# pascalPost/turbomesh

Hardware: AMD Instinct MI355X
Metric: nodes smoothed/sec (elliptic sweeps, 4096^2 blocks) + achieved HBM GB/s (higher is better)
Workload: dtype f64

## Files before the change

turbomesh_amd/csrc/tm_kernels.h:

```cpp
#pragma once
#include <hip/hip_runtime.h>
#include <cstdint>
#include "tm_edge_types.h"
#include <vector>

namespace tmh {

enum ApplyMode : int {
    MODE_RAW = 0,
    MODE_SCALED = 1,
    MODE_RESID = 2,
    MODE_RELAX = 3,
    MODE_DIAG_COPY = 4,
    MODE_DIAG_SUM9 = 5,
    MODE_DIAG_NOSTORE = 6,
    MODE_DIAG_NOLOAD = 7,
    MODE_DIAG_MATH = 8,
    MODE_MG_RESID = 9,
    MODE_MG_SMOOTH = 10,
    MODE_MG_FIRST2 = 11
};
enum DotMode : int {
    DOT_NONE = 0,
    DOT_AUX = 1,
// ... 29 lines not shown
int apply_block_nwg(int ni, int nj, int rows = 0);
int apply_block_nwg_overlap(int ni, int nj, int rows = 0);
void tune_apply(int rows_per_chunk, int unroll, int pipe, int nt);
hipError_t launch_apply_block(const ApplyBlock& a, int mode, int dot, hipStream_t stream);
constexpr int APPLY_BATCH_MAX = 8;
struct ApplyBatch {
    ApplyBlock b[APPLY_BATCH_MAX];
    int RI[APPLY_BATCH_MAX], nSG[APPLY_BATCH_MAX], nRC[APPLY_BATCH_MAX];
    int start[APPLY_BATCH_MAX];
    int n;
};
hipError_t launch_apply_blocks(const ApplyBlock* blocks, int n, int mode, int dot, hipStream_t stream);

struct Relax2Block {
    const double2* in;
    double2* mid;
    double2* out;
    int ni, nj;
    double omega;
    double* partials;
    const int32_t* border;
    int nborder;
    int store_nt = 1;
    int dyn;
};
bool relax2_supported(int ni, int nj);
int relax2_rows_per_chunk(int ni, int nj);
int relax2_block_nwg(int ni, int nj, int rows_per_chunk);
std::vector<int32_t> relax2_border_tiles(int ni, int nj, int rows_per_chunk, int dyn);
enum Relax2Subset { R2_ALL = 0, R2_BORDER = 1, R2_INSIDE_A = 2, R2_INSIDE_B = 3, R2_INSIDE = 4 };
constexpr long long QUEUE_WAIT_TICKS = 30LL * 100000000LL;
constexpr long long QUEUE_SELF_TEST_TICKS = 500000LL;
struct QueueWait {
    const uint32_t* counter = nullptr;
    uint32_t target = 0;
    uint32_t* error = nullptr;
    long long limit_ticks = QUEUE_WAIT_TICKS;
};
hipError_t launch_relax2_block(const Relax2Block& a, int rows_per_chunk, int dot, int subset, hipStream_t stream, size_t lds_bytes = 0,
                               const QueueWait* wait = nullptr);
struct Relax2Batch {
    Relax2Block b[8];
    int RI[8], nSG[8], nRC[8], start[8];
    int n;
};
hipError_t launch_relax2_blocks(const Relax2Block* blocks, const int* rows_per_chunk, int n, int dot, int subset, hipStream_t stream,
                                size_t lds_bytes = 0, const QueueWait* wait = nullptr);
void tune_fuse_rows(int rows);
bool relax3_supported(int ni, int nj);
int relax3_rows_per_chunk(int ni, int nj);
void relax3_rows_for_launch(const int* ni, const int* nj, int n, int* rows, bool beside_chain);
int relax3_block_nwg(int ni, int nj, int rows_per_chunk);
hipError_t launch_relax3_blocks(const Relax2Block* blocks, const int* rows_per_chunk, int n, int dot, hipStream_t stream);

hipError_t launch_edge_levels3(const FusedLevelsDev& F, const EdgeRowsDev& e1, const EdgeRowsDev& e2, const EdgeRowsDev& e3, const double2* x, double2* m,
                               double2* m2, double2* out, const double2* pq, double omega, int dot, double* partials ,
                               hipStream_t stream);
hipError_t launch_edge_rows(const EdgeRowsDev& e, const double2* in, const double2* xk, const double2* pq, const double2* aux,
                            double2* out, double omega, int mode, int dot, double* partials, hipStream_t stream, uint32_t* signal = nullptr);
hipError_t launch_apply_edge_blocks(const ApplyBlock* blocks, int n, int mode, int dot, const EdgeRowsDev& e, const double2* in, const double2* xk,
                                    const double2* pq, const double2* aux, double2* out, double* edge_partials, hipStream_t stream);
constexpr int VK_NONE = 0, VK_S = 1, VK_P = 2, VK_R = 3, VK_S2 = 4, VK_PRO = 5;
struct VirtualIn {
    int kind;
    const double2 *in, *in2, *in3, *aux;
    double2* pout;
    const double2* in4 = nullptr;
    double2* rout = nullptr;
    double2* uio = nullptr;
};
hipError_t launch_apply_virtual(const ApplyBlock* blocks, int n, const EdgeRowsDev& e, const VirtualIn& V, const double2* xk, const double2* pq, double2* out,
                                double* edge_partials, const LazyScalars& scal, hipStream_t stream, bool overlap = false);
hipError_t launch_edge_rhs(const EdgeRowsDev& e, const double2* xk, const double2* pq, double2* rhs_out, int scaled,
                           double* partials , hipStream_t stream);

hipError_t launch_queue_signal(uint32_t* counter, hipStream_t stream);
hipError_t launch_queue_wait(const uint32_t* counter, uint32_t target, uint32_t* error, hipStream_t stream, long long limit_ticks = QUEUE_WAIT_TICKS);
hipError_t launch_queue_signal_wait(uint32_t* counter, const uint32_t* other, uint32_t target, uint32_t* error, hipStream_t stream,
                                    long long limit_ticks = QUEUE_WAIT_TICKS);

hipError_t launch_assemble_interior(const double2* xk, const double2* pq, int ni, int nj, const int32_t* row_ptr ,
                                    double* vx, double* vy, hipStream_t stream);
hipError_t launch_assemble_edge(const EdgeRowsDev& e, const double2* xk, const double2* pq, const int32_t* row_ptr, double* vx, double* vy, hipStream_t stream);
hipError_t launch_csr_product(int64_t n, const int32_t* row_ptr, const int32_t* col, const double* vx, const double* vy, const double2* in, double2* out,
                              hipStream_t stream);
hipError_t launch_delay_us(double us, hipStream_t stream);

hipError_t launch_finalize(const double* partials, int nwg, double* red, hipStream_t stream);

struct KrylovScalars {
    double rho[2], rho_old[2], alpha[2], omega[2], beta[2];
    double tol2[2];
    double rr[2];
    double rr0[2];
    int32_t done[2];
    int32_t early[2];
    int32_t iters;
    int32_t _pad;
};
constexpr int VEC_BLOCK = 256;
int vec_nwg(int64_t n);
enum ScalarStep : int { STEP_INIT = 0, STEP_SIGMA = 1, STEP_SS = 2, STEP_TSTT = 3, STEP_RHO = 4, STEP_TOL = 5, STEP_SS_TSTT = 6, STEP_INIT2 = 7, STEP_A2 = 8, STEP_B2 = 9 };
hipError_t launch_scalar_update(KrylovScalars* S, const double* red, int step, hipStream_t stream, double rtol = 0.0, double atol = 0.0);
hipError_t launch_finalize_scalar(const double* partials, int nwg, double* red, KrylovScalars* S, int step, hipStream_t stream, double rtol = 0.0,
                                  double atol = 0.0);
struct LazyStep {
// ... 106 lines not shown
```

turbomesh_amd/csrc/tm_kernels.hip:

```cpp
#include "tm_kernels.h"
#include "tm_devutil.hpp"
#include "tm_refmath.h"
#include <cstdlib>
#include <type_traits>

namespace tmh {

__device__ __forceinline__ double lane_prev(double edge, double v) {
    int2 o = __builtin_bit_cast(int2, edge), s = __builtin_bit_cast(int2, v), r;
    r.x = __builtin_amdgcn_update_dpp(o.x, s.x, 0x138 , 0xf, 0xf, false);
    r.y = __builtin_amdgcn_update_dpp(o.y, s.y, 0x138, 0xf, 0xf, false);
    return __builtin_bit_cast(double, r);
}
__device__ __forceinline__ double lane_next(double edge, double v) {
    int2 o = __builtin_bit_cast(int2, edge), s = __builtin_bit_cast(int2, v), r;
    r.x = __builtin_amdgcn_update_dpp(o.x, s.x, 0x130 , 0xf, 0xf, false);
    r.y = __builtin_amdgcn_update_dpp(o.y, s.y, 0x130, 0xf, 0xf, false);
    return __builtin_bit_cast(double, r);
}
__device__ __forceinline__ double2 lane_prev(double2 edge, double2 v) { return make_double2(lane_prev(edge.x, v.x), lane_prev(edge.y, v.y)); }
__device__ __forceinline__ double2 lane_next(double2 edge, double2 v) { return make_double2(lane_next(edge.x, v.x), lane_next(edge.y, v.y)); }

__device__ __forceinline__ double2 lane_prev0(double2 v) {
    int4 s = __builtin_bit_cast(int4, v), r;
// ... 838 lines not shown
            __builtin_amdgcn_raw_buffer_store_b128(__builtin_bit_cast(v4i32, o), out_rsrc,
                                                   static_cast<int>(row_live ? lane_off + static_cast<unsigned>((i - t.i0) * nj * 16) : OOB_VOFFSET), 0,
                                                   (NT & 1) ? 2 : 0);
            if (DOT == DOT_DELTA) {
                if (!(live_lane && row_live)) d3 = zero;
                accumulate<DOT_DELTA>(acc, S2[A1].c, o, d3);
            }
        }
#pragma unroll
        for (int u = 0; u < U; ++u) pc[u] = pn[u];
    };
    static_assert(U == 3, "the phases below assume three steps per group");
    group(0, 0);
    group(U, 1);
    for (int tb = 2 * U; tb < nsteps; tb += U) group(tb, 2);
}

template <int DOT, int U, int NT, bool W1>
__device__ __forceinline__ void relax3_tile(const Relax2Block& a, int RI, int nSG, int nRC, int bid) {
    const int lane = threadIdx.x & 63;
    const int wave = threadIdx.x >> 6;
    const int total = nSG * nRC;
    const int q8 = total >> 3, rem = total & 7, xcd = bid & 7, k8 = bid >> 3;
    const int logical = (xcd < rem) ? xcd * (q8 + 1) + k8 : rem * (q8 + 1) + (xcd - rem) * q8 + k8;
    const int rc = logical / nSG;
    const int sg = logical - rc * nSG;
    const int ni = a.ni, nj = a.nj;
    Relax2Tile t;
    t.c0 = (sg * 4 + wave) * R3_W;
    t.c = t.c0 - R3_H + lane;
    t.out_lane = (lane >= R3_H) && (lane < 64 - R3_H) && (t.c >= 1) && (t.c <= nj - 2);
    t.i0 = 1 + rc * RI;
    t.i1 = min(t.i0 + RI, ni - 1);
    double acc[MAX_PARTIALS] = {0.0, 0.0, 0.0, 0.0};
    if (t.c0 <= nj - 2 && t.i0 < t.i1) {
        const bool inside = (t.c0 - R3_H >= 1) && (t.c0 - R3_H + 63 <= nj - 2) && (t.i0 - 3 >= 1) && (t.i1 + 2 <= ni - 2);
        if (inside) relax3_strip<DOT, U, NT, W1, true>(a, t, acc);
        else relax3_strip<DOT, U, NT, W1, false>(a, t, acc);
    }
    if (DOT != DOT_NONE) block_partials<256, dot_columns(DOT)>(acc, a.partials + static_cast<size_t>(logical) * MAX_PARTIALS);
}
template <int DOT, int U, int NT, bool W1>
__global__ __launch_bounds__(256, TM_R3_WAVES) void k_relax3(Relax2Block a, int RI, int nSG, int nRC) {
    relax3_tile<DOT, U, NT, W1>(a, RI, nSG, nRC, blockIdx.x);
}
template <int DOT, int U, int NT, bool W1>
__global__ __launch_bounds__(256) void k_relax3_batch(Relax2Batch B) {
    int k = 0;
#pragma unroll
    for (int q = 1; q < APPLY_BATCH_MAX; ++q)
        if (q < B.n && static_cast<int>(blockIdx.x) >= B.start[q]) k = q;
    relax3_tile<DOT, U, NT, W1>(B.b[k], B.RI[k], B.nSG[k], B.nRC[k], static_cast<int>(blockIdx.x) - B.start[k]);
}
static int g_fuse3_rows = 0;
void relax3_rows_for_launch(const int* ni, const int* nj, int n, int* rows, bool beside_chain) {
    static const int forced = [] { const char* e = std::getenv("TM_FUSE3_ROWS"); return e ? std::atoi(e) : 0; }();
    if (forced > 0 || g_fuse3_rows > 0) {
        for (int k = 0; k < n; ++k) rows[k] = std::max(1, std::min(forced > 0 ? forced : g_fuse3_rows, ni[k] - 2));
        return;
    }
    static int slots = 0;
    if (slots == 0) {
        int dev = 0, cus = 0;
        if (hipGetDevice(&dev) != hipSuccess || hipDeviceGetAttribute(&cus, hipDeviceAttributeMultiprocessorCount, dev) != hipSuccess || cus <= 0) cus = 256;
        slots = 3 * cus;
    }
    static const int heights[] = {38, 26, 14, 8};
    const long need = static_cast<long>(slots) * (beside_chain ? 9 : 6);
    int RI = 8;
    for (const int h : heights) {
        long total = 0;
        for (int k = 0; k < n; ++k) {
            const int nstrips = (nj[k] - 1 + R3_W - 1) / R3_W, nSG = (nstrips + 3) / 4, interior = ni[k] - 2, r = std::max(1, std::min(h, interior));
            total += static_cast<long>(nSG) * ((interior + r - 1) / r);
        }
        RI = h;
        if (total * 10 >= need) break;
    }
    for (int k = 0; k < n; ++k) rows[k] = std::max(1, std::min(RI, ni[k] - 2));
}
int relax3_rows_per_chunk(int ni, int nj) {
    int r = 0;
    relax3_rows_for_launch(&ni, &nj, 1, &r, false);
    return r;
}
bool relax3_supported(int ni, int nj) { return ni >= 7 && nj >= 7 && nj <= (1 << 20); }
int relax3_block_nwg(int ni, int nj, int RI) {
    const int nstrips = (nj - 1 + R3_W - 1) / R3_W;
    return ((nstrips + 3) / 4) * ((ni - 2 + RI - 1) / RI);
}
hipError_t launch_relax3_blocks(const Relax2Block* blocks, const int* rows_per_chunk, int n, int dot, hipStream_t st) {
    for (int first = 0; first < n; first += APPLY_BATCH_MAX) {
        Relax2Batch B;
        B.n = 0;
        int total = 0;
        bool w1 = true;
        const bool nts = blocks[first].store_nt != 0;
        for (int k = first; k < n && B.n < APPLY_BATCH_MAX; ++k) {
            const int q = B.n++;
            B.b[q] = blocks[k];
            B.RI[q] = rows_per_chunk[k];
            B.nSG[q] = ((blocks[k].nj - 1 + R3_W - 1) / R3_W + 3) / 4;
            B.nRC[q] = (blocks[k].ni - 2 + B.RI[q] - 1) / B.RI[q];
            B.start[q] = total;
            total += B.nSG[q] * B.nRC[q];
            w1 = w1 && blocks[k].omega == 1.0;
        }
        for (int q = B.n; q < APPLY_BATCH_MAX; ++q) B.start[q] = total;
        if (total == 0) continue;
        const dim3 grid(total), block(256);
#define TM_R3(KERNEL, ...)                                                                                                   \
    do {                                                                                                                     \
        if (dot == DOT_DELTA) {                                                                                              \
            if (w1 && nts) hipLaunchKernelGGL((KERNEL<DOT_DELTA, R3_U, 1, true>), grid, block, 0, st, __VA_ARGS__);          \
            else if (w1) hipLaunchKernelGGL((KERNEL<DOT_DELTA, R3_U, 0, true>), grid, block, 0, st, __VA_ARGS__);            \
            else hipLaunchKernelGGL((KERNEL<DOT_DELTA, R3_U, 1, false>), grid, block, 0, st, __VA_ARGS__);                   \
        } else {                                                                                                             \
            if (w1 && nts) hipLaunchKernelGGL((KERNEL<DOT_NONE, R3_U, 1, true>), grid, block, 0, st, __VA_ARGS__);           \
            else if (w1) hipLaunchKernelGGL((KERNEL<DOT_NONE, R3_U, 0, true>), grid, block, 0, st, __VA_ARGS__);             \
            else hipLaunchKernelGGL((KERNEL<DOT_NONE, R3_U, 1, false>), grid, block, 0, st, __VA_ARGS__);                    \
        }                                                                                                                    \
    } while (0)
        static const bool force_batch = [] { const char* e = std::getenv("TM_R3_FORCE_BATCH"); return e && std::atoi(e) != 0; }();
        if (B.n == 1 && !force_batch) TM_R3(k_relax3, B.b[0], B.RI[0], B.nSG[0], B.nRC[0]);
        else TM_R3(k_relax3_batch, B);
#undef TM_R3
        const hipError_t rc = hipGetLastError();
        if (rc != hipSuccess) return rc;
    }
    return hipSuccess;
}

constexpr int MG_RST_W = 58;
struct MgMetric {
    double G11, G22, mhG12, m2D, D, rinv;
};
__device__ __forceinline__ MgMetric mg_metric(double2 dxi, double2 det) {
    MgMetric m;
    m.G11 = fma(dxi.x, dxi.x, dxi.y * dxi.y);
    m.G22 = fma(det.x, det.x, det.y * det.y);
    const double G12 = fma(dxi.x, det.x, dxi.y * det.y);
    m.D = m.G11 + m.G22;
    m.m2D = -2.0 * m.D;
    m.mhG12 = -0.5 * G12;
    m.rinv = recip_diag(m.D, m.m2D);
    return m;
}
template <bool HAS_PQ>
__device__ __forceinline__ double2 mg_scaled_row(const MgMetric& g, const Row3& m, const Row3& c, const Row3& p, double P, double Q) {
    double ax = p.c.x + m.c.x, ay = p.c.y + m.c.y;
    double bx = c.h.x, by = c.h.y;
    if (HAS_PQ) {
        const double hP = 0.5 * P, hQ = 0.5 * Q;
        ax = fma(hP, p.c.x - m.c.x, ax);
        ay = fma(hP, p.c.y - m.c.y, ay);
        bx = fma(hQ, c.e.x, bx);
        by = fma(hQ, c.e.y, by);
    }
    const double kx = p.e.x - m.e.x;
    const double ky = p.e.y - m.e.y;
    double sx = g.G22 * ax, sy = g.G22 * ay;
    sx = fma(g.G11, bx, sx);
    sy = fma(g.G11, by, sy);
    sx = fma(g.m2D, c.c.x, sx);
    sy = fma(g.m2D, c.c.y, sy);
    sx = fma(g.mhG12, kx, sx);
    sy = fma(g.mhG12, ky, sy);
    return make_double2(sx * g.rinv, sy * g.rinv);
}

template <int KIND, bool HAS_PQ, bool PRO, bool RST, int U>
__device__ __forceinline__ void mg_pair_strip(const MgPairArgs& a, const Relax2Tile& t) {
    static_assert(!RST || KIND == 1, "the restriction rides behind the residual");
    const int ni = a.ni, nj = a.nj;
    const int cc = min(max(t.c, 0), nj - 1);
    const double2 zero = make_double2(0.0, 0.0);
    auto at = [&](int row) { return static_cast<size_t>(min(max(row, 0), ni - 1)) * nj + cc; };
    const bool perim_col = (t.c <= 0) || (t.c >= nj - 1);
    const bool col_in = (t.c >= 1) && (t.c <= nj - 2);
    const int nrows = t.i1 - t.i0;
    const __amdgpu_buffer_rsrc_t out_rsrc = __builtin_amdgcn_make_buffer_rsrc(a.out + static_cast<size_t>(t.i0) * nj, 0, nrows * nj * 16, 0x00020000);
    const __amdgpu_buffer_rsrc_t out2_rsrc =
        __builtin_amdgcn_make_buffer_rsrc((KIND == 1 ? a.out2 : a.out) + static_cast<size_t>(t.i0) * nj, 0, nrows * nj * 16, 0x00020000);
// ... 1804 lines not shown
```

turbomesh_amd/csrc/tm_smoother.cpp:

```cpp
#include "tm_smoother.hpp"
#include "tm_api_util.hpp"
#include "tm_ilu.hpp"
#include "tm_refine.hpp"
#include "tm_quality_dev.hpp"
#include <algorithm>
#include <atomic>
#include <chrono>
#include <cmath>
#include <cstdio>
#include <cstdlib>
#include <cstring>
#include <map>
#include <unordered_map>

namespace tmh {

void hip_check(hipError_t e, const char* what) {
    if (e != hipSuccess) throw TmError(TM_E_HIP, std::string(what) + ": " + hipGetErrorString(e));
}
#define HIPCHK(x) hip_check((x), #x)

std::atomic<int> g_multirank_handles{0};
tm_log_fn g_log_sink = nullptr;
void* g_log_ctx = nullptr;
// ... 400 lines not shown
        return 0;
    };
    apply_rows = shortest_rows(false);
    vk_overlap = vk_able && lp.n_owned >= 50000 && lp.n_owned <= 12000000;
    if (vk_overlap && launch_wgs(apply_rows, false) <= 256 && launch_wgs(shortest_rows(true), true) > 256) vk_overlap = false;
    if (const char* e = std::getenv("TM_VK_OVERLAP")) vk_overlap = vk_able && std::atoi(e) != 0;
    if (vk_overlap) apply_rows = shortest_rows(true);
    if (vk_able && !apply_rows && lp.owned_blocks.size() > 1) apply_rows = 24;
    if (!apply_rows && opt.inner == TM_INNER_RELAX) apply_rows = 6;
    if (const char* e = std::getenv("TM_APPLY_ROWS")) apply_rows = std::max(0, std::atoi(e));
    poff.clear();
    int off = 0;
    for (int64_t b : lp.owned_blocks) {
        poff.push_back(off);
        off += apply_block_nwg(static_cast<int>(topo.ni[b]), static_cast<int>(topo.nj[b]), apply_rows);
    }
    poff_edge = off;
    off += edge_wg;
    nwg_apply = off;
    if (fuse_pairs) {
        poff2.clear();
        rows2.clear();
        int off2 = 0;
        for (int64_t b : lp.owned_blocks) {
            const int bi = static_cast<int>(topo.ni[b]), bj = static_cast<int>(topo.nj[b]);
            poff2.push_back(off2);
            rows2.push_back(relax2_rows_per_chunk(bi, bj));
            off2 += relax2_block_nwg(bi, bj, rows2.back());
            const std::vector<int32_t> ids = relax2_border_tiles(bi, bj, rows2.back(), dyn_mask[poff2.size() - 1]);
            border_n.push_back(static_cast<int>(ids.size()));
            border_ids.push_back(static_cast<const int32_t*>(upload_table(ids.data(), ids.size() * 4)));
        }
        poff2_edge = off2;
        nwg_apply2 = off2 + edge_nf.nwg;
    }
    pipelined_single = fuse_pairs && !(has_hooks && (lp.send_ids.size() > 0 || !lp.ghost_gid.empty())) && edge_nf.nrows > 0 && lp.n_owned >= (1 << 21);
    if (const char* e = std::getenv("TM_SINGLE_PIPELINED")) pipelined_single = pipelined_single && std::atoi(e) != 0;
    fuse_triples = fuse_pairs && edge_nf.nrows == 0 && !(has_hooks && (!lp.send_ids.empty() || !lp.ghost_gid.empty()));
    if (const char* e = std::getenv("TM_FUSE_3")) fuse_triples = fuse_triples && std::atoi(e) != 0;
    if (fuse_triples || triples_coupled) {
        poff3.clear();
        rows3.clear();
        int off3 = 0;
        rows3 = relax3_rows_of_owned_blocks();
        for (size_t k = 0; k < lp.owned_blocks.size(); ++k) {
            const int64_t b = lp.owned_blocks[k];
            const int bi = static_cast<int>(topo.ni[b]), bj = static_cast<int>(topo.nj[b]);
            if (!relax3_supported(bi, bj)) fuse_triples = false;
            poff3.push_back(off3);
            off3 += relax3_block_nwg(bi, bj, rows3[k]);
        }
        nwg_apply3 = off3;
    }
    nwg_vec = vec_nwg(n_owned);
    const int nwg3_all = fuse_triples ? nwg_apply3 : (triples_coupled ? nwg_apply3 + std::max(edge_L[2].nwg, fused_levels.nstrips) : 0);
    if (vk_overlap) {
        int off_ov = 0;
        for (int64_t b : lp.owned_blocks) {
            poff_ov.push_back(off_ov);
            off_ov += apply_block_nwg_overlap(static_cast<int>(topo.ni[b]), static_cast<int>(topo.nj[b]), apply_rows);
        }
        poff_edge_ov = off_ov;
        nwg_apply_ov = off_ov + edge.nwg;
    }
    if (vk_able && std::max(nwg_apply, nwg_apply_ov) <= 512) nwg_vec = std::min(nwg_vec, 512);
    lazy = !has_hooks && opt.inner != TM_INNER_RELAX && std::max(std::max(nwg_apply, nwg_apply_ov), nwg_vec) <= 512 && !(opt.flags & TM_OPT_EAGER_SCALARS);
    const int nwg_refine = refine() ? csr_nwg(n_owned) : 0;
    const uint64_t npart = static_cast<uint64_t>(std::max(std::max(std::max(std::max(std::max(nwg_apply, nwg_apply_ov), nwg_apply2), nwg3_all), nwg_vec), nwg_refine)) * MAX_PARTIALS;
    fuse_s = !has_hooks && opt.inner == TM_INNER_BICGSTAB && !(opt.flags & TM_OPT_EAGER_SCALARS);
    fuse_p = fuse_s;
    if (const char* e = std::getenv("TM_FUSE_P")) fuse_p = fuse_p && std::atoi(e) != 0;
    fuse2 = fuse_p;
    if (const char* e = std::getenv("TM_FUSE_2")) fuse2 = fuse2 && std::atoi(e) != 0;
    if (fuse_p) {
        p_alt = vec();
        v_alt = vec();
    }
    if (fuse2) r_alt = vec();
    const int rows = static_cast<int>(npart / MAX_PARTIALS);
    const struct {
        const char* what;
        int nwg;
    } producers[] = {{"operator", nwg_apply},
                     {"operator (overlapping strips)", nwg_apply_ov},
                     {"sweep pairs", nwg_apply2},
                     {"sweep triples", nwg3_all},
                     {"vector kernels", nwg_vec},
                     {"GMRES Gram-Schmidt", (opt.inner == TM_INNER_GMRES || reference()) ? vec_nwg(n_owned) : 0},
                     {"perimeter-row right-hand side", opt.inner != TM_INNER_RELAX ? edge.nwg : 0},
                     {"refinement step", nwg_refine}};
    if (std::getenv("TM_DEBUG_RUNS"))
        std::fprintf(stderr, "[tm] partial-sum rows: %d allocated; operator %d, overlapping strips %d, pairs %d, triples %d, vector kernels %d (vec_nwg %d)\n", rows,
                     nwg_apply, nwg_apply_ov, nwg_apply2, nwg3_all, nwg_vec, vec_nwg(n_owned));
    for (const auto& q : producers)
        if (q.nwg > rows)
            throw TmError(TM_E_HIP, std::string("internal: the ") + q.what + " launch has " + std::to_string(q.nwg) + " workgroups, the partial-sum buffer " +
                                        std::to_string(rows) + " rows");
    return npart;
}

void Smoother::alloc_reductions(uint64_t npart) {
    partials_guard = false;
    if (const char* e = std::getenv("TM_PARTIALS_GUARD")) partials_guard = std::atoi(e) != 0;
    const uint64_t nguard = partials_guard ? GUARD_DOUBLES : 0;
    for (int k = 0; k < (lazy ? 3 : 1); ++k) part_buf[k] = arena.alloc_n<double>(npart + nguard);
    partials = part_buf[0];
    red = arena.alloc_n<double>(MAX_PARTIALS + nguard);
    if (partials_guard) {
// ... 932 lines not shown
    }
    return rows;
}

void Smoother::ensure_side() {
    if (side) return;
    int least = 0, greatest = 0;
    HIPCHK(hipDeviceGetStreamPriorityRange(&least, &greatest));
    HIPCHK(hipStreamCreateWithPriority(&side, hipStreamNonBlocking, greatest));
    HIPCHK(hipEventCreateWithFlags(&ev_to_side, hipEventDisableTiming));
    HIPCHK(hipEventCreateWithFlags(&ev_to_main, hipEventDisableTiming));
    HIPCHK(hipEventCreateWithFlags(&ev_inside[0], hipEventDisableTiming));
    HIPCHK(hipEventCreateWithFlags(&ev_inside[1], hipEventDisableTiming));
    if (pair_sync_events) queue_ordering = ORDER_EVENTS_REQUESTED;
    else queue_ordering = queue_self_test() ? ORDER_COUNTERS : ORDER_EVENTS_SELF_TEST;
}

bool Smoother::queue_self_test() {
    HIPCHK(hipStreamSynchronize(stream));
    HIPCHK(hipStreamSynchronize(side));
    uint32_t* a = sync_flags + 8;
    uint32_t* b = sync_flags + 9;
    uint32_t* err = sync_flags + 10;
    HIPCHK(hipMemsetAsync(sync_flags + 8, 0, sizeof(uint32_t) * 4, stream));
    HIPCHK(hipStreamSynchronize(stream));
    HIPCHK(launch_queue_signal_wait(a, b, 1u, err, stream, QUEUE_SELF_TEST_TICKS));
    HIPCHK(launch_queue_signal_wait(b, a, 1u, err, side, QUEUE_SELF_TEST_TICKS));
    HIPCHK(hipStreamSynchronize(stream));
    HIPCHK(hipStreamSynchronize(side));
    uint32_t h[4] = {0, 0, 0, 0};
    HIPCHK(hipMemcpy(h, sync_flags + 8, sizeof(h), hipMemcpyDeviceToHost));
    return h[2] == 0u && h[0] == 1u && h[1] == 1u;
}

bool Smoother::use_counters() {
    if (queue_ordering == ORDER_EVENTS_REQUESTED || queue_ordering == ORDER_EVENTS_SELF_TEST) return false;
    if (g_multirank_handles.load() > 1) {
        queue_ordering = ORDER_EVENTS_SHARED_PROCESS;
        return false;
    }
    queue_ordering = ORDER_COUNTERS;
    return true;
}

void Smoother::warm_transport() {
    if (transport_warm) return;
    transport_warm = true;
    if (!(has_hooks && (n_send > 0 || n_ghost > 0))) return;
    exchange(X, side);
    exchange_finish(side);
    HIPCHK(hipStreamSynchronize(side));
}

void Smoother::relax_triple(bool want_partials) {
    const int dot = want_partials ? DOT_DELTA : DOT_NONE;
    std::vector<Relax2Block> blocks(lp.owned_blocks.size());
    for (size_t k = 0; k < lp.owned_blocks.size(); ++k) {
        const int64_t b = lp.owned_blocks[k];
        const int64_t ls = lp.local_start[k];
        Relax2Block& a = blocks[k];
        a.in = X + ls;
        a.mid = nullptr;
        a.out = U + ls;
        a.ni = static_cast<int>(topo.ni[b]);
        a.nj = static_cast<int>(topo.nj[b]);
        a.omega = opt.omega;
        a.dyn = 0;
        a.store_nt = relax2_store_nt ? 1 : 0;
        a.border = nullptr;
        a.nborder = 0;
        a.partials = partials + static_cast<size_t>(poff3[k]) * MAX_PARTIALS;
    }
    profiled([&]() { HIPCHK(launch_relax3_blocks(blocks.data(), rows3.data(), static_cast<int>(blocks.size()), dot, stream)); }, true, stream);
    std::swap(X, U);
}

void Smoother::relax_triples_coupled(uint64_t ntriples, bool want_partials_last) {
    ensure_side();
    const bool use_flags = use_counters();
    uint32_t* chain_done = sync_flags;
    uint32_t* inside_done = sync_flags + 1;
    uint32_t* sync_err = sync_flags + 2;
    if (use_flags) HIPCHK(hipMemsetAsync(sync_flags, 0, sizeof(uint32_t) * 4, stream));
    fence(stream, side, ev_to_side);
    warm_transport();
    std::vector<Relax2Block> blocks(lp.owned_blocks.size());
    for (uint64_t q = 0; q < ntriples; ++q) {
        const int dot = (q + 1 == ntriples && want_partials_last) ? DOT_DELTA : DOT_NONE;
        for (size_t k = 0; k < lp.owned_blocks.size(); ++k) {
            const int64_t b = lp.owned_blocks[k];
            const int64_t ls = lp.local_start[k];
            Relax2Block& a = blocks[k];
            a.in = X + ls;
            a.mid = nullptr;
            a.out = U + ls;
            a.ni = static_cast<int>(topo.ni[b]);
            a.nj = static_cast<int>(topo.nj[b]);
            a.omega = opt.omega;
            a.dyn = dyn_mask[k];
            a.store_nt = relax2_store_nt ? 1 : 0;
            a.border = nullptr;
            a.nborder = 0;
            a.partials = partials + static_cast<size_t>(poff3[k]) * MAX_PARTIALS;
        }
        if (q > 0) {
            if (use_flags) HIPCHK(launch_queue_signal_wait(inside_done, chain_done, static_cast<uint32_t>(q), sync_err, stream));
            else HIPCHK(hipStreamWaitEvent(stream, ev_to_main, 0));
        }
        profiled([&]() { HIPCHK(launch_relax3_blocks(blocks.data(), rows3.data(), static_cast<int>(blocks.size()), dot, stream)); }, true, stream);
        if (!use_flags) HIPCHK(hipEventRecord(ev_inside[q & 1], stream));
        if (q > 0) {
            if (use_flags) HIPCHK(launch_queue_signal_wait(chain_done, inside_done, static_cast<uint32_t>(q), sync_err, side));
            else HIPCHK(hipStreamWaitEvent(side, ev_inside[(q - 1) & 1], 0));
        }
        exchange(X, side);
        exchange_finish(side);
        if (levels_fused) {
            HIPCHK(launch_edge_levels3(fused_levels, edge_L[0], edge_L[1], edge_L[2], X, M, M2, U, PQ, opt.omega, dot,
                                       partials + static_cast<size_t>(nwg_apply3) * MAX_PARTIALS, side));
        } else {
            HIPCHK(launch_edge_rows(edge_L[0], X, X, PQ, nullptr, M, opt.omega, MODE_RELAX, DOT_NONE, partials, side));
            HIPCHK(launch_edge_rows(edge_L[1], M, M, PQ, nullptr, M2, opt.omega, MODE_RELAX, DOT_NONE, partials, side));
            HIPCHK(launch_edge_rows(edge_L[2], M2, M2, PQ, nullptr, U, opt.omega, MODE_RELAX, dot, partials + static_cast<size_t>(nwg_apply3) * MAX_PARTIALS, side));
        }
        if (q + 1 < ntriples && !use_flags) HIPCHK(hipEventRecord(ev_to_main, side));
        std::swap(X, U);
// ... 53 lines not shown
            w.counter = inside_done;
            w.target = inside_upto;
            w.error = sync_err;
            relax2_launch(R2_BORDER, true, dot, side, &w);
        } else {
            if (inside_upto > 0) wait_inside(inside_upto);
            relax2_launch(R2_BORDER, true, dot, side);
        }
    };
    int dot = (npairs == 1 && want_partials_last) ? DOT_DELTA : DOT_NONE;
    fence(stream, side, ev_to_side);
    warm_transport();
    exchange_on_side(X);
    edge_on_side(e1, X, M, DOT_NONE);
    relax2_launch(R2_INSIDE, false, dot);
    if (!use_flags || npairs == 1) signal_inside();
    border_pass(0, dot);
    for (uint64_t k = 0; k < npairs; ++k) {
        const bool announce = k + 1 < npairs;
        if (use_flags && announce) {
            edge_on_side(edge_nf, M, U, dot, border_done);
            n_border += 1;
        } else {
            edge_on_side(edge_nf, M, U, dot);
            if (announce) signal_border();
        }
        std::swap(X, U);
        if (k + 1 == npairs) {
            fence(side, stream, ev_to_main);
            break;
        }
        dot = (k + 2 == npairs && want_partials_last) ? DOT_DELTA : DOT_NONE;
        if (use_flags) {
            HIPCHK(launch_queue_signal_wait(inside_done, border_done, n_border, sync_err, stream));
            n_inside += 1;
        } else {
            wait_border();
        }
        relax2_launch(R2_INSIDE, false, dot);
        if (!use_flags) signal_inside();
        exchange_on_side(X);
        edge_on_side(e1, X, M, DOT_NONE);
        border_pass(static_cast<uint32_t>(k + 1), dot);
    }
    if (use_flags) {
        HIPCHK(hipMemcpyAsync(h_flags, sync_flags, sizeof(uint32_t) * 4, hipMemcpyDeviceToHost, stream));
        flags_pending = true;
    }
}

void Smoother::relax_sweeps(uint64_t n, tm_stats& st) {
    int last_nwg = nwg_apply;
    uint64_t k = 0;
    if ((fuse_triples || triples_coupled) && n >= 3) {
        const uint64_t ntriples = n / 3;
        if (fuse_triples) {
            for (uint64_t q = 0; q < ntriples; ++q) relax_triple(q + 1 == ntriples && n % 3 == 0);
            last_nwg = nwg_apply3;
        } else {
            relax_triples_coupled(ntriples, n % 3 == 0);
            last_nwg = nwg_apply3 + (levels_fused ? fused_levels.nstrips : edge_L[2].nwg);
        }
        k = 3 * ntriples;
        st.operator_sweeps += k;
        outer_done += k;
    }
    if (fuse_pairs && n - k >= 2) {
        const uint64_t npairs = (n - k) / 2;
        const bool last_is_pair = (n - k) % 2 == 0;
        if ((has_hooks && (n_send > 0 || n_ghost > 0)) || pipelined_single) {
            relax_pairs_pipelined(npairs, last_is_pair);
        } else {
            for (uint64_t q = 0; q < npairs; ++q) relax_pair(q + 1 == npairs && last_is_pair);
        }
        k += 2 * npairs;
        st.operator_sweeps += 2 * npairs;
        outer_done += 2 * npairs;
        last_nwg = nwg_apply2;
    }
    for (; k < n; ++k) {
        last_nwg = nwg_apply;
        if (white && outer_done > 0) white_launch(1);
        apply(X, U, MODE_RELAX, DOT_DELTA, nullptr, X, opt.omega);
        std::swap(X, U);
        st.operator_sweeps += 1;
        outer_done += 1;
    }
    if (profile && prof_open) {
        profile_close(stream);
        prof_phase = 0;
    }
    if (n) {
        reduce(last_nwg);
        HIPCHK(hipMemcpyAsync(h_red, red, sizeof(double) * MAX_PARTIALS, hipMemcpyDeviceToHost, stream));
        sync();
        if (flags_pending) {
            flags_pending = false;
            const bool timed_out = h_flags[2] != 0 || h_flags[6] != 0;
            h_flags[2] = h_flags[6] = 0;
            if (timed_out) throw TmError(TM_E_HIP, "a device-side dependency between the interior pass and the chain of a sweep pair / triple was not met within its time limit");
        }
        st.last_dx2 = h_red[0];
        st.last_dy2 = h_red[1];
        st.last_residual = (h_red[0] + h_red[1]) * (h_red[0] + h_red[1]);
        st.scaled_residual_rms = std::sqrt((h_red[0] + h_red[1]) / (2.0 * static_cast<double>(dof_global))) / opt.omega;
    }
}

void Smoother::iterate(uint64_t iterations, tm_stats* stats) {
    const auto t0 = std::chrono::steady_clock::now();
    tm_stats st;
    std::memset(&st, 0, sizeof(st));
    const tm_log_fn sink = g_log_sink;
    if (opt.inner == TM_INNER_RELAX && !sink) {
        relax_sweeps(iterations, st);
        st.outer_iterations = iterations;
    } else {
        for (uint64_t n = 0; n < iterations; ++n) {
// ... 279 lines not shown
```

turbomesh_amd/csrc/tm_smoother.hpp:

```cpp
#pragma once
#include "../../include/tm_hip.h"
#include <cstdlib>
#include "tm_edge_tables.hpp"
#include "tm_kernels.h"
#include "tm_multigrid.hpp"
#include "tm_plan.hpp"
#include <cmath>
#include <atomic>
#include <memory>
#include <string>
#include <functional>
#include <vector>

namespace tmh {

struct TmError : std::runtime_error {
    int code;
    TmError(int c, const std::string& m) : std::runtime_error(m), code(c) {}
};
void hip_check(hipError_t e, const char* what);
extern std::atomic<int> g_multirank_handles;
extern tm_log_fn g_log_sink;
extern void* g_log_ctx;

// ... 41 lines not shown
    std::vector<BlockMG> mg;
    bool use_mg = false;
    bool mg_perimeter_step = false;
    bool mg_dirichlet = false;
    std::vector<hipStream_t> mg_streams;
    std::vector<hipEvent_t> mg_join;
    hipEvent_t mg_fork = nullptr;
    int mg_perimeter_sweeps = 2;
    void precondition(const double2* in, double2* out);
    void precondition_probe_host(const double* f, double* z, double* f_after);
    double2* M = nullptr;
    double2* M2 = nullptr;
    bool fuse_pairs = false;
    bool relax2_store_nt = true;
    bool pair_sync_events = false;
    size_t inside_lds = 0;
    EdgeRowsDev edge;
    std::vector<double> h_rhs;
    struct RhsTable {
        double* dev = nullptr;
        std::vector<const double*> src;
    };
    std::vector<RhsTable> rhs_tables;
    EdgeRowsDev edge_nf;
    EdgeRowsDev edge_nf_g;
    std::vector<int> dyn_mask;
    std::vector<const int32_t*> border_ids;
    std::vector<int> border_n;
    void prefill_fixed();
    double* partials = nullptr;
    double* red = nullptr;
    KrylovScalars* S = nullptr;
    KrylovScalars* h_S = nullptr;
    bool pipelined_poll = false, poll_open = false;
    KrylovScalars* h_poll[2] = {nullptr, nullptr};
    hipEvent_t ev_poll[2] = {nullptr, nullptr};
    uint64_t poll_it[2] = {0, 0}, poll_iters = 0;
    int poll_slot = 0;
    int poll_done(uint64_t it, bool final);
    double stall_best[2] = {0.0, 0.0};
    uint64_t stall_since = 0, stall_window = 4000;
    bool stalled = false;
    double* h_red = nullptr;
    bool vk_overlap = false;
    std::vector<int> poff_ov;
    int poff_edge_ov = 0, nwg_apply_ov = 0;
    std::vector<int> poff;
    int poff_edge = 0, nwg_apply = 0, nwg_vec = 0;
    std::vector<int> poff2, rows2;
    int poff2_edge = 0, nwg_apply2 = 0;
    std::vector<int> poff3, rows3;
    int nwg_apply3 = 0;
    bool fuse_triples = false;
    bool triples_coupled = false;
    EdgeRowsDev edge_L[3];
    bool levels_fused = false;
    FusedLevelsDev fused_levels;
    bool pipelined_single = false;
    int32_t* d_send_ids = nullptr;
    double2* d_send_buf = nullptr;
    int64_t n_send = 0;
    bool white = false;
    ConnShifts white_le{};
    uint64_t outer_done = 0;
    int profile = 0;
    std::vector<hipEvent_t> ev_start, ev_stop;
    size_t ev_used = 0;
    uint64_t prof_launches = 0;
    uint64_t prof_timed = 0;
    uint64_t prof_open = 0;
    uint64_t prof_phase = 0;
    void profile_close(hipStream_t on);
    void profile_read(double* ms_total, uint64_t* launches, uint64_t* timed);

    void create(const tm_mesh_desc* mesh, const tm_solver_opt* o, const tm_control_fn* c, const tm_comm_hooks* h, void* strm,
                bool measure);
    void upload(const tm_mesh_desc* mesh);
    void download(const tm_mesh_desc* mesh);
    void iterate(uint64_t iterations, tm_stats* stats);
    bool iterate_until(uint64_t max_iterations, double tol, tm_stats* stats);
    bool iterate_until_update(uint64_t max_iterations, double tol, tm_stats* stats);
    double stop_tol = 0.0;
    void apply_host(const double* in_xy, double* out_xy, int scaled);
    uint64_t assemble_csr_host(int32_t* Ap, int32_t* Ai, double* Ax_x, double* Ax_y, uint64_t nnz_capacity);
    void apply_reference_host(const double* in_xy, double* out_xy);
    struct AssembledCsr {
        int32_t *p = nullptr, *i = nullptr;
        double *vx = nullptr, *vy = nullptr;
        uint64_t nnz = 0;
        std::vector<int32_t> h_p, h_i;
    } csr;
    void csr_build_pattern();
    void csr_fill_values();
    void csr_release();
    void csr_free();
    void rhs_host(double* rhs_xy);
    void residual_host(const double* xy, double* r_xy);
    void control_function_host(double* pq);
    void export_soa_host(int64_t block, double* x, double* y, double* p, double* q);
    void* export_buf = nullptr;
    size_t export_bytes = 0;
    QualityDev* qdev = nullptr;
    void quality_host(tm_quality* per_block, tm_quality* total);
    void quality_field_host(int64_t block, double* out);

    void exchange(double2* vec, hipStream_t on = nullptr);
// ... 38 lines not shown
    void flush_pending();
    LazyScalars scalars_for();
    void white_launch(int update);
    void sync();
    void ensure_tmp();

    double2* gm_V = nullptr;
    GmresScalars* gm_S = nullptr;
    GmresScalars* h_gm = nullptr;

    struct ReferenceSolve;
    ReferenceSolve* ref = nullptr;
    void reference_create();
    double2* ref_b = nullptr;
    double2 *rf_r = nullptr, *rf_d = nullptr, *rf_dinv = nullptr;
    uint32_t refine_steps = 0;
    double refine_rel[2] = {0.0, 0.0};
    double refine_rtol = 0.0;
    uint64_t refine_iterations = 0;
    bool refine() const { return (opt.flags & TM_OPT_REFINE) != 0; }
    uint64_t inner_counts[2] = {0, 0};

   private:
    struct Selection;
    bool reference() const { return opt.inner == TM_INNER_REFERENCE_GMRES; }
    double2* vec() { return arena.alloc_n<double2>(static_cast<uint64_t>(n_local)); }
    void resolve_options(const tm_mesh_desc* mesh, const tm_solver_opt* o, const tm_control_fn* c, const tm_comm_hooks* h, bool measure);
    void plan_mesh(const tm_mesh_desc* mesh, const tm_comm_hooks* h, bool measure);
    void alloc_vectors(const tm_mesh_desc* mesh, bool measure);
    void decide_schedule();
    void* upload_table(const void* src, uint64_t bytes);
    RunTable make_table(const Selection& sel, EdgeRowsDev& e);
    void build_row_tables();
    uint64_t size_launches();
    void alloc_reductions(uint64_t npart);
    void finish_create(const tm_mesh_desc* mesh);
    int picard_bicgstab(tm_stats& st);
    int picard_gmres(tm_stats& st);
    int picard_reference(tm_stats& st);
    void refine_solution();
    uint64_t correct_bicgstab(const double2* rhs, double2* d);
    uint64_t correct_gmres(const double2* rhs, double2* d);
    int picard_solve(tm_stats& st) {
        const uint64_t before = st.inner_iterations;
        if (opt.inner == TM_INNER_REFERENCE_GMRES) return picard_reference(st);
        const int rc = opt.inner == TM_INNER_GMRES ? picard_gmres(st) : picard_bicgstab(st);
        inner_counts[0] = inner_counts[1] = st.inner_iterations - before;
        return rc;
    }
    void relax_sweeps(uint64_t n, tm_stats& st);
    void relax_pair(bool want_partials);
    std::vector<int> relax3_rows_of_owned_blocks() const;
    void relax_triple(bool want_partials);
    void relax_triples_coupled(uint64_t ntriples, bool want_partials_last);
    void profiled(const std::function<void()>& launch, bool counts = true, hipStream_t on = nullptr);
    void relax2_launch(int subset, bool counts, int dot, hipStream_t on = nullptr, const QueueWait* wait = nullptr);
};

inline bool triples_wanted(const tm_solver_opt& o, const tm_control_fn& c) {
    if (o.inner != TM_INNER_RELAX || c.kind != TM_CF_LAPLACE || (o.flags & TM_OPT_SINGLE_SWEEP)) return false;
    if (const char* e = std::getenv("TM_TRIPLES_COUPLED")) return std::atoi(e) != 0;
    return true;
}
int rccl_hooks_allow_triples(const tm_comm_hooks* h);

constexpr uint64_t AUTO_MG_MIN_BLOCK_NODES = 100000;
constexpr uint64_t AUTO_MG_MIN_LONE_BLOCK_NODES = 1000;
constexpr double AUTO_MG_MAX_ASPECT_SPREAD = 1.0;

inline double default_rtol(double nodes) {
    const double r = 7.5e-9 / (nodes > 1.0 ? nodes : 1.0);
    return r > 1e-14 ? 1e-14 : (r < 1e-16 ? 1e-16 : r);
}
inline uint64_t default_max_inner(double nodes) {
    const double k = 12.0 * std::sqrt(nodes > 1.0 ? nodes : 1.0);
    return k > 10000.0 ? static_cast<uint64_t>(k) : 10000u;
}

}

struct tm_smoother {
    tmh::Smoother impl;
};
```

Measured before the change: 447.1 billion.

## Add four-sweep temporally fused relaxation kernel with depth-4 halo walls

Adds a kernel that fuses four Jacobi-style relaxation sweeps per launch. Each wave keeps a sliding register window of intermediate rows, and the strip overlaps its neighbours by a 4-column halo. The smoother uses it by default when triples are enabled, the blocks are large enough and the block shape is supported, then falls back to triples and pairs for the remaining sweeps. This cuts HBM round trips per sweep compared with three-sweep fusion, at the cost of more redundant halo computation, fewer useful lanes per wave (56 of 64), and higher register pressure from the extra stage windows.

```diff
diff --git a/turbomesh_amd/csrc/tm_kernels.h b/turbomesh_amd/csrc/tm_kernels.h
--- a/turbomesh_amd/csrc/tm_kernels.h
+++ b/turbomesh_amd/csrc/tm_kernels.h
@@ -105,6 +105,10 @@
 void relax3_rows_for_launch(const int* ni, const int* nj, int n, int* rows, bool beside_chain);
 int relax3_block_nwg(int ni, int nj, int rows_per_chunk);
 hipError_t launch_relax3_blocks(const Relax2Block* blocks, const int* rows_per_chunk, int n, int dot, hipStream_t stream);
+bool relax4_supported(int ni, int nj);
+void relax4_rows_for_launch(const int* ni, const int* nj, int n, int* rows);
+int relax4_block_nwg(int ni, int nj, int rows_per_chunk);
+hipError_t launch_relax4_blocks(const Relax2Block* blocks, const int* rows_per_chunk, int n, int dot, hipStream_t stream);
 
 hipError_t launch_edge_levels3(const FusedLevelsDev& F, const EdgeRowsDev& e1, const EdgeRowsDev& e2, const EdgeRowsDev& e3, const double2* x, double2* m,
                                double2* m2, double2* out, const double2* pq, double omega, int dot, double* partials ,
diff --git a/turbomesh_amd/csrc/tm_kernels.hip b/turbomesh_amd/csrc/tm_kernels.hip
--- a/turbomesh_amd/csrc/tm_kernels.hip
+++ b/turbomesh_amd/csrc/tm_kernels.hip
@@ -914,6 +914,116 @@
         if (q < B.n && static_cast<int>(blockIdx.x) >= B.start[q]) k = q;
     relax3_tile<DOT, U, NT, W1>(B.b[k], B.RI[k], B.nSG[k], B.nRC[k], static_cast<int>(blockIdx.x) - B.start[k]);
 }
+constexpr int R4_L = 4;
+constexpr int R4_W = 64 - 2 * R4_L;
+template <int L, int DOT, int U, int NT, bool W1, bool INSIDE>
+__device__ __forceinline__ void relaxn_strip(const Relax2Block& a, const Relax2Tile& t, double (&acc)[MAX_PARTIALS]) {
+    static_assert(U == 3 && L >= 3, "three steps per group; the windows rotate by renaming");
+    constexpr int STEADY = (2 * (L - 1) + 2) / 3;
+    const int ni = a.ni, nj = a.nj;
+    const int cc = INSIDE ? t.c : min(max(t.c, 0), nj - 1);
+    const double2* in_col = a.in + cc;
+    const int last_row = INSIDE ? t.i1 + L - 1 : ni - 1;
+    auto load_in = [&](int row) { return in_col[static_cast<size_t>(INSIDE ? min(row, last_row) : min(max(row, 0), last_row)) * nj]; };
+    const bool perim_col = !INSIDE && ((t.c <= 0) || (t.c >= nj - 1));
+    const int nrows = t.i1 - t.i0;
+    const __amdgpu_buffer_rsrc_t out_rsrc = __builtin_amdgcn_make_buffer_rsrc(a.out + static_cast<size_t>(t.i0) * nj, 0, nrows * nj * 16, 0x00020000);
+    const unsigned lane_off = t.out_lane ? static_cast<unsigned>(cc) * 16u : OOB_VOFFSET;
+    const double2 zero = make_double2(0.0, 0.0);
+    const int r0 = t.i0 - (L - 2);
+
+    Row3 A[3], S[L - 1][3];
+    double2 pc[U], pn[U];
+    {
+        const double2 a0 = load_in(r0 - 2), a1 = load_in(r0 - 1);
+#pragma unroll
+        for (int u = 0; u < U; ++u) pc[u] = load_in(r0 + u);
+        A[0] = make_row(a0);
+        A[1] = make_row(a1);
+        A[2].c = A[2].e = A[2].h = zero;
+#pragma unroll
+        for (int k = 0; k < L - 1; ++k) S[k][0] = S[k][1] = S[k][2] = A[2];
+    }
+    const int nsteps = nrows + 2 * (L - 1);
+    auto group = [&](const int tb, const int phase) {
+#pragma unroll
+        for (int u = 0; u < U; ++u) pn[u] = load_in(r0 + tb + U + u);
+#pragma unroll
+        for (int u = 0; u < U; ++u) {
+            const int A0 = u % 3, A1 = (u + 1) % 3, A2 = (u + 2) % 3;
+            const int r = r0 + tb + u;
+            const int s = U * phase + u;
+            A[A2] = make_row(pc[u]);
+            double2 d = zero;
+            double2 v = relax_row<W1>(A[A0], A[A1], A[A2], a.omega, d);
+            if (!INSIDE && (perim_col || r - 1 <= 0 || r - 1 >= ni - 1)) v = A[A1].c;
+            S[0][A2] = make_row(v);
+#pragma unroll
+            for (int k = 2; k < L; ++k) {
+                if (phase >= STEADY || s >= 2 * (k - 1)) {
+                    v = relax_row<W1>(S[k - 2][A0], S[k - 2][A1], S[k - 2][A2], a.omega, d);
+                    if (!INSIDE && (perim_col || r - k <= 0 || r - k >= ni - 1)) v = S[k - 2][A1].c;
+                    S[k - 1][A2] = make_row(v);
+                }
+            }
+            double2 dl = zero, o = zero;
+            if (phase >= STEADY || s >= 2 * (L - 1)) o = relax_row<W1>(S[L - 2][A0], S[L - 2][A1], S[L - 2][A2], a.omega, dl);
+            const int i = r - L;
+            const bool row_live = (i >= t.i0) && (i < t.i1);
+            __builtin_amdgcn_raw_buffer_store_b128(__builtin_bit_cast(v4i32, o), out_rsrc,
+                                                   static_cast<int>(row_live ? lane_off + static_cast<unsigned>((i - t.i0) * nj * 16) : OOB_VOFFSET), 0,
+                                                   (NT & 1) ? 2 : 0);
+            if (DOT == DOT_DELTA) {
+                if (!(t.out_lane && row_live)) dl = zero;
+                accumulate<DOT_DELTA>(acc, S[L - 2][A1].c, o, dl);
+            }
+        }
+#pragma unroll
+        for (int u = 0; u < U; ++u) pc[u] = pn[u];
+    };
+    static_assert(STEADY == 2, "two warm-up groups are peeled below");
+    group(0, 0);
+    group(U, 1);
+    for (int tb = 2 * U; tb < nsteps; tb += U) group(tb, STEADY);
+}
+
+template <int L, int DOT, int U, int NT, bool W1>
+__device__ __forceinline__ void relaxn_tile(const Relax2Block& a, int RI, int nSG, int nRC, int bid) {
+    constexpr int W = 64 - 2 * L;
+    const int lane = threadIdx.x & 63;
+    const int wave = threadIdx.x >> 6;
+    const int total = nSG * nRC;
+    const int q8 = total >> 3, rem = total & 7, xcd = bid & 7, k8 = bid >> 3;
+    const int logical = (xcd < rem) ? xcd * (q8 + 1) + k8 : rem * (q8 + 1) + (xcd - rem) * q8 + k8;
+    const int rc = logical / nSG;
+    const int sg = logical - rc * nSG;
+    const int ni = a.ni, nj = a.nj;
+    Relax2Tile t;
+    t.c0 = (sg * 4 + wave) * W;
+    t.c = t.c0 - L + lane;
+    t.out_lane = (lane >= L) && (lane < 64 - L) && (t.c >= 1) && (t.c <= nj - 2);
+    t.i0 = 1 + rc * RI;
+    t.i1 = min(t.i0 + RI, ni - 1);
+    double acc[MAX_PARTIALS] = {0.0, 0.0, 0.0, 0.0};
+    if (t.c0 <= nj - 2 && t.i0 < t.i1) {
+        const bool inside = (t.c0 - L >= 1) && (t.c0 - L + 63 <= nj - 2) && (t.i0 - L >= 1) && (t.i1 + L - 1 <= ni - 2);
+        if (inside) relaxn_strip<L, DOT, U, NT, W1, true>(a, t, acc);
+        else relaxn_strip<L, DOT, U, NT, W1, false>(a, t, acc);
+    }
+    if (DOT != DOT_NONE) block_partials<256, dot_columns(DOT)>(acc, a.partials + static_cast<size_t>(logical) * MAX_PARTIALS);
+}
+template <int DOT, int U, int NT, bool W1>
+__global__ __launch_bounds__(256) void k_relax4(Relax2Block a, int RI, int nSG, int nRC) {
+    relaxn_tile<R4_L, DOT, U, NT, W1>(a, RI, nSG, nRC, blockIdx.x);
+}
+template <int DOT, int U, int NT, bool W1>
+__global__ __launch_bounds__(256) void k_relax4_batch(Relax2Batch B) {
+    int k = 0;
+#pragma unroll
+    for (int q = 1; q < APPLY_BATCH_MAX; ++q)
+        if (q < B.n && static_cast<int>(blockIdx.x) >= B.start[q]) k = q;
+    relaxn_tile<R4_L, DOT, U, NT, W1>(B.b[k], B.RI[k], B.nSG[k], B.nRC[k], static_cast<int>(blockIdx.x) - B.start[k]);
+}
 static int g_fuse3_rows = 0;
 void relax3_rows_for_launch(const int* ni, const int* nj, int n, int* rows, bool beside_chain) {
     static const int forced = [] { const char* e = std::getenv("TM_FUSE3_ROWS"); return e ? std::atoi(e) : 0; }();
@@ -951,7 +1061,8 @@
     const int nstrips = (nj - 1 + R3_W - 1) / R3_W;
     return ((nstrips + 3) / 4) * ((ni - 2 + RI - 1) / RI);
 }
-hipError_t launch_relax3_blocks(const Relax2Block* blocks, const int* rows_per_chunk, int n, int dot, hipStream_t st) {
+static hipError_t launch_fixed_wall_blocks(int depth, const Relax2Block* blocks, const int* rows_per_chunk, int n, int dot, hipStream_t st) {
+    const int W = 64 - 2 * depth;
     for (int first = 0; first < n; first += APPLY_BATCH_MAX) {
         Relax2Batch B;
         B.n = 0;
@@ -962,7 +1073,7 @@
             const int q = B.n++;
             B.b[q] = blocks[k];
             B.RI[q] = rows_per_chunk[k];
-            B.nSG[q] = ((blocks[k].nj - 1 + R3_W - 1) / R3_W + 3) / 4;
+            B.nSG[q] = ((blocks[k].nj - 1 + W - 1) / W + 3) / 4;
             B.nRC[q] = (blocks[k].ni - 2 + B.RI[q] - 1) / B.RI[q];
             B.start[q] = total;
             total += B.nSG[q] * B.nRC[q];
@@ -984,13 +1095,59 @@
         }                                                                                                                    \
     } while (0)
         static const bool force_batch = [] { const char* e = std::getenv("TM_R3_FORCE_BATCH"); return e && std::atoi(e) != 0; }();
-        if (B.n == 1 && !force_batch) TM_R3(k_relax3, B.b[0], B.RI[0], B.nSG[0], B.nRC[0]);
-        else TM_R3(k_relax3_batch, B);
+        const bool lone = B.n == 1 && !force_batch;
+        if (depth == R4_L) {
+            if (lone) TM_R3(k_relax4, B.b[0], B.RI[0], B.nSG[0], B.nRC[0]);
+            else TM_R3(k_relax4_batch, B);
+        } else {
+            if (lone) TM_R3(k_relax3, B.b[0], B.RI[0], B.nSG[0], B.nRC[0]);
+            else TM_R3(k_relax3_batch, B);
+        }
 #undef TM_R3
         const hipError_t rc = hipGetLastError();
         if (rc != hipSuccess) return rc;
     }
     return hipSuccess;
+}
+hipError_t launch_relax3_blocks(const Relax2Block* blocks, const int* rows_per_chunk, int n, int dot, hipStream_t st) {
+    return launch_fixed_wall_blocks(3, blocks, rows_per_chunk, n, dot, st);
+}
+
+void relax4_rows_for_launch(const int* ni, const int* nj, int n, int* rows) {
+    static const int forced = [] { const char* e = std::getenv("TM_FUSE4_ROWS"); return e ? std::atoi(e) : 0; }();
+    if (forced > 0) {
+        for (int k = 0; k < n; ++k) rows[k] = std::max(1, std::min(forced, ni[k] - 2));
+        return;
+    }
+    static int slots = 0;
+    if (slots == 0) {
+        int dev = 0, cus = 0;
+        if (hipGetDevice(&dev) != hipSuccess || hipDeviceGetAttribute(&cus, hipDeviceAttributeMultiprocessorCount, dev) != hipSuccess || cus <= 0) cus = 256;
+        slots = 3 * cus;
+    }
+    static const int heights[] = {54, 42, 30, 18, 6};
+    const long need = static_cast<long>(slots) * 6;
+    int RI = 6;
+    for (const int h : heights) {
+        long total = 0;
+        for (int k = 0; k < n; ++k) {
+            const int nstrips = (nj[k] - 1 + R4_W - 1) / R4_W, nSG = (nstrips + 3) / 4, interior = ni[k] - 2, r = std::max(1, std::min(h, interior));
+            total += static_cast<long>(nSG) * ((interior + r - 1) / r);
+        }
+        RI = h;
+        if (total * 10 >= need) break;
+    }
+    for (int k = 0; k < n; ++k) rows[k] = std::max(1, std::min(RI, ni[k] - 2));
+}
+bool relax4_supported(int ni, int nj) { return ni >= 2 * R4_L + 1 && nj >= 2 * R4_L + 1 && nj <= (1 << 20); }
+int relax4_block_nwg(int ni, int nj, int RI) {
+    const int nstrips = (nj - 1 + R4_W - 1) / R4_W;
+    return ((nstrips + 3) / 4) * ((ni - 2 + RI - 1) / RI);
+}
+hipError_t launch_relax4_blocks(const Relax2Block* blocks, const int* rows_per_chunk, int n, int dot, hipStream_t st) {
+    for (int k = 0; k < n; ++k)
+        if (blocks[k].dyn != 0) return hipErrorInvalidValue;
+    return launch_fixed_wall_blocks(R4_L, blocks, rows_per_chunk, n, dot, st);
 }
 
 constexpr int MG_RST_W = 58;
diff --git a/turbomesh_amd/csrc/tm_smoother.cpp b/turbomesh_amd/csrc/tm_smoother.cpp
--- a/turbomesh_amd/csrc/tm_smoother.cpp
+++ b/turbomesh_amd/csrc/tm_smoother.cpp
@@ -476,8 +476,38 @@
         }
         nwg_apply3 = off3;
     }
+    fuse_quads = fuse_triples;
+    bool quads_forced = false;
+    if (const char* e = std::getenv("TM_FUSE_4")) {
+        fuse_quads = fuse_quads && std::atoi(e) != 0;
+        quads_forced = std::atoi(e) != 0;
+    }
+    nwg_apply4 = 0;
+    if (fuse_quads) {
+        std::vector<int> bi, bj;
+        for (size_t first = 0; first < lp.owned_blocks.size(); first += APPLY_BATCH_MAX) {
+            int64_t nodes = 0;
+            for (size_t k = first; k < std::min<size_t>(first + APPLY_BATCH_MAX, lp.owned_blocks.size()); ++k) nodes += topo.ni[lp.owned_blocks[k]] * topo.nj[lp.owned_blocks[k]];
+            if (nodes < QUAD_MIN_NODES && !quads_forced) fuse_quads = false;
+        }
+        for (int64_t b : lp.owned_blocks) {
+            bi.push_back(static_cast<int>(topo.ni[b]));
+            bj.push_back(static_cast<int>(topo.nj[b]));
+            if (!relax4_supported(bi.back(), bj.back())) fuse_quads = false;
+        }
+        poff4.clear();
+        rows4.assign(bi.size(), 1);
+        for (size_t first = 0; first < rows4.size(); first += APPLY_BATCH_MAX)
+            relax4_rows_for_launch(bi.data() + first, bj.data() + first, static_cast<int>(std::min<size_t>(APPLY_BATCH_MAX, rows4.size() - first)), rows4.data() + first);
+        int off4 = 0;
+        for (size_t k = 0; k < rows4.size(); ++k) {
+            poff4.push_back(off4);
+            off4 += relax4_block_nwg(bi[k], bj[k], rows4[k]);
+        }
+        nwg_apply4 = fuse_quads ? off4 : 0;
+    }
     nwg_vec = vec_nwg(n_owned);
-    const int nwg3_all = fuse_triples ? nwg_apply3 : (triples_coupled ? nwg_apply3 + std::max(edge_L[2].nwg, fused_levels.nstrips) : 0);
+    const int nwg3_all = std::max(nwg_apply4, fuse_triples ? nwg_apply3 : (triples_coupled ? nwg_apply3 + std::max(edge_L[2].nwg, fused_levels.nstrips) : 0));
     if (vk_overlap) {
         int off_ov = 0;
         for (int64_t b : lp.owned_blocks) {
@@ -1516,8 +1546,11 @@
     HIPCHK(hipStreamSynchronize(side));
 }
 
-void Smoother::relax_triple(bool want_partials) {
+void Smoother::relax_triple(bool want_partials) { relax_fixed_walls(3, want_partials); }
+void Smoother::relax_quad(bool want_partials) { relax_fixed_walls(4, want_partials); }
+void Smoother::relax_fixed_walls(int depth, bool want_partials) {
     const int dot = want_partials ? DOT_DELTA : DOT_NONE;
+    const std::vector<int>& poffd = depth == 4 ? poff4 : poff3;
     std::vector<Relax2Block> blocks(lp.owned_blocks.size());
     for (size_t k = 0; k < lp.owned_blocks.size(); ++k) {
         const int64_t b = lp.owned_blocks[k];
@@ -1533,9 +1566,10 @@
         a.store_nt = relax2_store_nt ? 1 : 0;
         a.border = nullptr;
         a.nborder = 0;
-        a.partials = partials + static_cast<size_t>(poff3[k]) * MAX_PARTIALS;
-    }
-    profiled([&]() { HIPCHK(launch_relax3_blocks(blocks.data(), rows3.data(), static_cast<int>(blocks.size()), dot, stream)); }, true, stream);
+        a.partials = partials + static_cast<size_t>(poffd[k]) * MAX_PARTIALS;
+    }
+    if (depth == 4) profiled([&]() { HIPCHK(launch_relax4_blocks(blocks.data(), rows4.data(), static_cast<int>(blocks.size()), dot, stream)); }, true, stream);
+    else profiled([&]() { HIPCHK(launch_relax3_blocks(blocks.data(), rows3.data(), static_cast<int>(blocks.size()), dot, stream)); }, true, stream);
     std::swap(X, U);
 }
 
@@ -1695,18 +1729,26 @@
 void Smoother::relax_sweeps(uint64_t n, tm_stats& st) {
     int last_nwg = nwg_apply;
     uint64_t k = 0;
-    if ((fuse_triples || triples_coupled) && n >= 3) {
-        const uint64_t ntriples = n / 3;
+    if (fuse_quads && n >= 4) {
+        const uint64_t nquads = n / 4 - (n % 4 == 1 ? 1 : 0);
+        for (uint64_t q = 0; q < nquads; ++q) relax_quad(q + 1 == nquads && n == 4 * nquads);
+        k = 4 * nquads;
+        if (nquads) last_nwg = nwg_apply4;
+        st.operator_sweeps += k;
+        outer_done += k;
+    }
+    if ((fuse_triples || triples_coupled) && n - k >= 3) {
+        const uint64_t ntriples = (n - k) / 3;
         if (fuse_triples) {
-            for (uint64_t q = 0; q < ntriples; ++q) relax_triple(q + 1 == ntriples && n % 3 == 0);
+            for (uint64_t q = 0; q < ntriples; ++q) relax_triple(q + 1 == ntriples && (n - k) % 3 == 0);
             last_nwg = nwg_apply3;
         } else {
             relax_triples_coupled(ntriples, n % 3 == 0);
             last_nwg = nwg_apply3 + (levels_fused ? fused_levels.nstrips : edge_L[2].nwg);
         }
-        k = 3 * ntriples;
-        st.operator_sweeps += k;
-        outer_done += k;
+        k += 3 * ntriples;
+        st.operator_sweeps += 3 * ntriples;
+        outer_done += 3 * ntriples;
     }
     if (fuse_pairs && n - k >= 2) {
         const uint64_t npairs = (n - k) / 2;
diff --git a/turbomesh_amd/csrc/tm_smoother.hpp b/turbomesh_amd/csrc/tm_smoother.hpp
--- a/turbomesh_amd/csrc/tm_smoother.hpp
+++ b/turbomesh_amd/csrc/tm_smoother.hpp
@@ -117,6 +117,10 @@
     std::vector<int> poff3, rows3;
     int nwg_apply3 = 0;
     bool fuse_triples = false;
+    std::vector<int> poff4, rows4;
+    int nwg_apply4 = 0;
+    bool fuse_quads = false;
+    static constexpr int64_t QUAD_MIN_NODES = 8000000;
     bool triples_coupled = false;
     EdgeRowsDev edge_L[3];
     bool levels_fused = false;
@@ -261,6 +265,8 @@
     void relax_pair(bool want_partials);
     std::vector<int> relax3_rows_of_owned_blocks() const;
     void relax_triple(bool want_partials);
+    void relax_quad(bool want_partials);
+    void relax_fixed_walls(int depth, bool want_partials);
     void relax_triples_coupled(uint64_t ntriples, bool want_partials_last);
     void profiled(const std::function<void()>& launch, bool counts = true, hipStream_t on = nullptr);
     void relax2_launch(int subset, bool counts, int dot, hipStream_t on = nullptr, const QueueWait* wait = nullptr);
```

New measurement: 468.7 billion, median of 6. +4.8%, better.
